# huang-yh/GaussianFormer

Measured on AMD Instinct MI355X. Metric: Gaussians/sec splatted into 200×200×16×18 voxel grid (fwd), higher is better.
Workload: dtype f32

## Files before the change

### gaussianformer_amd/csrc/splat_bwd_mfma.hip

```cpp
#include <algorithm>


#include "gf_common.hpp"
#include "splat_mfma.hpp"

#ifndef GF_TIMELINE
#define GF_TIMELINE 0
#endif

namespace gf {

constexpr int kBwdBigTableAt = kLongWords, kBwdBigTable = (kBwdBigCap - kBwdBigTableAt - 1) / 3;
static_assert(kBwdBigTableAt >= kWRow && kBwdBigTable >= 64, "the table sits past the layout words in use");

struct BwdMArgs {
    const float *pts;
    const float *records;
    const uint2 *boxes;
    const unsigned long long *bitmask;
    const float *out_grad;
    float *rows;
    float *means_grad, *opa_grad, *sem_grad, *cov_grad;
    const uint32_t *state;
    uint32_t *tile_counters;
// ... 218 lines not shown
            if (off >= per_col) { off -= per_col; col += 1; }
        }
    };

    uint32_t *ctr = a.tile_counters + 64 * xcd;
    const int nchunk = (a.nwords + 63) >> 6;
    int local = (int)(blockIdx.x >> 3);
    while (true) {
        const int logical = local;
        const int qs = (int)__umulhi((uint32_t)logical, m_ps);
        if (!(local < per_xcd && 8 * qs + xcd < a.nsx * a.nsy)) break;
        uint32_t claimed = 0u;
        const int s = 8 * qs + xcd, r = logical - qs * per_super;
        const int srow = a.nsy == 1 ? s : (int)__umulhi((uint32_t)s, m_nsy), scol = s - srow * a.nsy;
        const int Xw = srow * kSuper + 4 * (r & 1), Y0 = scol * kSuper + 4 * ((r >> 1) & 1), Zw = 8 * (r >> 2);
        if (Xw < a.H && Y0 < a.W) {
#if GF_TIMELINE
            unsigned long long tl[8] = {(unsigned long long)wall_clock64(), 0, 0, 0, 0, 0, 0, 0};
#endif
            const uint32_t published_len = use_lists ? a.list_len[s] : 0u;
            request_unit(s, Xw, Y0, Zw);
            if (dl_by16) asm volatile("s_waitcnt vmcnt(9)" ::: "memory");
            else asm volatile("s_waitcnt vmcnt(36)" ::: "memory");
#if GF_TIMELINE
            tl[1] = wall_clock64();
#endif
            int list_len = 0, qlen = 0, qhead = 0, npend = 0;
            int c = 0, sg = 0;
            bool have_boxes = false;
            const bool pub_unit = LONG ? (use_lists && published_len != 0xFFFFFFFFu) : use_lists;
            int pub_done = 0;
            bool pub_fetch = false;
            if (pub_unit) {
                list_len = min((int)published_len, kMList);
                c = nchunk;
                have_boxes = true;
            } else if (!LONG) {
                constexpr int kWDense = kMList;
                uint32_t *s_dw = s_u;
                unsigned long long *s_db = reinterpret_cast<unsigned long long *>(s_u + kWDense);
                constexpr int kWPer = (kWRow + 63) / 64;
                const int kw = nchunk;
                unsigned long long wd[kWPer];
                int mine = 0;
                int wlane = lane;
                asm volatile("" : "+v"(wlane));
                const int wbase = kw * wlane;
#pragma unroll
                for (int k = 0; k < kWPer; ++k) wd[k] = s_row[min(wbase + k, kWRow - 1)];
                static_assert(kWPer == 10, "operand list below");
                asm volatile("" : "+v"(wd[0]), "+v"(wd[1]), "+v"(wd[2]), "+v"(wd[3]), "+v"(wd[4]), "+v"(wd[5]), "+v"(wd[6]), "+v"(wd[7]),
                             "+v"(wd[8]), "+v"(wd[9]));
#pragma unroll
                for (int k = 0; k < kWPer; ++k) {
                    const int w = wbase + k;
                    wd[k] = (k < kw && w < a.nwords) ? wd[k] : 0ull;
                    mine += wd[k] != 0ull ? 1 : 0;
                }
                const int incl_nz = wave_incl_scan_dpp(mine);
                const int nd = __builtin_amdgcn_readlane(incl_nz, 63);
                if (nd <= kWDense) {
                    int p = incl_nz - mine;
#pragma unroll
                    for (int k = 0; k < kWPer; ++k) {
                        if (wd[k] != 0ull) {
                            s_dw[p] = (uint32_t)(wbase + k);
                            s_db[p] = wd[k];
// ... 754 lines not shown
```

### gaussianformer_amd/csrc/splat_fwd.hip

```cpp
#include <string.h>

#include <algorithm>

#include "gf_common.hpp"
#include "splat_mfma.hpp"

#ifndef GF_TIMELINE
#define GF_TIMELINE 0
#endif

namespace gf {

struct PrepArgs {
    const float *means3D;
    const int *means_int;
    const float *opacity;
    const float *semantics;
    const int *radii;
    const float *cov3D;
    const int *points_int;
    const float *pts;
    float *records;
    uint2 *boxes;
    unsigned long long *bitmask;
    uint32_t *verify_flags;
    int P, N, H, W, D, nwords, nrow, nsx, nsy, per_axis, variant, nprep_blocks, verify, prescale, exact_det, lattice;
    uint32_t *tile_counters;
    uint32_t tile_counter_init;
    uint32_t *unit_totals;
    uint32_t *unit_local;
    uint32_t *bwd_counters;
    uint32_t bwd_counter_init;
    uint32_t *gen_word;
    const uint32_t *gate_state;
    int range_theta_here;
    uint32_t *verdict_words;
    unsigned char *summary;
    int sum_pitch;
    uint32_t *range_flags;
};

constexpr int kPrepSuperChunk = 4096;

__device__ __forceinline__ void gaussian_box(const int *__restrict__ means_int, const int *__restrict__ radii,
                                             int per_axis, int g, int H, int W, int D, int lo[3], int hi[3])
{
    const int m0 = means_int[3 * g], m1 = means_int[3 * g + 1], m2 = means_int[3 * g + 2];
    int r0, r1, r2;
    if (per_axis) {
        r0 = radii[3 * g]; r1 = radii[3 * g + 1]; r2 = radii[3 * g + 2];
    } else {
        r0 = r1 = r2 = radii[g];
    }
    lo[0] = min(H, max(0, m0 - r0)); hi[0] = min(H, max(0, m0 + r0 + 1));
    lo[1] = min(W, max(0, m1 - r1)); hi[1] = min(W, max(0, m1 + r1 + 1));
    lo[2] = min(D, max(0, m2 - r2)); hi[2] = min(D, max(0, m2 + r2 + 1));
}

__device__ __forceinline__ float prob_kdet(float c0, float c1, float c2, float c3, float c4, float c5, int exact)
{
    float deter, kdet;
    prob_det_kdet(c0, c1, c2, c3, c4, c5, exact, deter, kdet);
    return kdet;
}

constexpr float kSemRangeMax = 64.f;

__device__ __forceinline__ uint32_t range_bits_of(const float *c, const float *sm, float opa, int r0, int r1, int r2, int H, int W,
                                                  int D, float lsx, float lsy, float lsz)
{
    const float ex = (float)(min(r0, H) + 3) * lsx, ey = (float)(min(r1, W) + 3) * lsy, ez = (float)(min(r2, D) + 5) * lsz;
    const float bound = 0.7213475f * (fabsf(c[0]) + fabsf(c[1]) + fabsf(c[2])) * (ex * ex + ey * ey + ez * ez);
// ... 75 lines not shown
                                         (double)pz[k] == p0z + (double)z[k] * sz);
                }
            }
        }
        if (first_round) {
            p0x = q0x; p0y = q0y; p0z = q0z;
            sx = a.H > 1 ? (double)q1x - p0x : 1.0;
            sy = a.W > 1 ? (double)q1y - p0y : 1.0;
            sz = a.D > 1 ? (double)q1z - p0z : 1.0;
        }
        if (a.lattice) {
            const float lx_ = fabsf((float)sx), ly_ = fabsf((float)sy), lz_ = fabsf((float)sz);
            const float zero[kC] = {0.f};
            if (has_g) rbits |= range_bits_of(c0, zero, 0.f, rr0, rr1, rr2, a.H, a.W, a.D, lx_, ly_, lz_) & kVerdictTheta;
#pragma nounroll
            for (int g = g0 + kVerifyBlocks * 64; g < a.P; g += kVerifyBlocks * 64) {
                const float *cv = a.cov3D + 6 * (size_t)g;
                const int r0 = a.radii[a.per_axis ? 3 * g : g], r1 = a.radii[a.per_axis ? 3 * g + 1 : g], r2 = a.radii[a.per_axis ? 3 * g + 2 : g];
                float c[6];
#pragma unroll
                for (int j = 0; j < 6; ++j) c[j] = cv[j];
                rbits |= range_bits_of(c, zero, 0.f, r0, r1, r2, a.H, a.W, a.D, lx_, ly_, lz_) & kVerdictTheta;
            }
        }
        const unsigned long long any = __builtin_amdgcn_ballot_w64(bad), any2 = __builtin_amdgcn_ballot_w64(bad_lattice),
                                 any3 = __builtin_amdgcn_ballot_w64((rbits & kVerdictTheta) != 0u);
        const uint32_t vbits = (any ? kVerdictPoint : 0u) | (any2 ? kVerdictLattice : 0u) | (any3 ? kVerdictTheta : 0u);
        if (lane == 0) a.verify_flags[vb] = vbits;
        if (a.verdict_words && vbits && lane == 0) atomicOr(a.verdict_words + verdict_slot_after(a.verdict_words[kVerdictA]), vbits);
        return;
    }
    if (a.tile_counters && blockIdx.x == 0 && threadIdx.x < 8) a.tile_counters[64 * threadIdx.x] = a.tile_counter_init;
    if (a.verdict_words && blockIdx.x == 0 && threadIdx.x == 0) a.verdict_words[kVerdictB] = a.verdict_words[kVerdictA] + 1u;
    const int word = blockIdx.x * WAVES + wave;
    const int g = word * 64 + lane;
    const bool valid = g < a.P;
    int lo[3] = {0, 0, 0}, hi[3] = {0, 0, 0};
    uint32_t range_bits = 0u;
    float lsx = 0.f, lsy = 0.f, lsz = 0.f;
    if (a.range_flags && a.range_theta_here) {
        const float p0x = a.pts[0], p0y = a.pts[1], p0z = a.pts[2];
        lsx = a.H > 1 ? fabsf(a.pts[3 * (size_t)a.W * a.D] - p0x) : 1.f;
        lsy = a.W > 1 ? fabsf(a.pts[3 * (size_t)a.D + 1] - p0y) : 1.f;
        lsz = a.D > 1 ? fabsf(a.pts[3 + 2] - p0z) : 1.f;
    }
    auto range_of = [&](const float *c, const float *sm, float opa, int r0, int r1, int r2) -> uint32_t {
        return range_bits_of(c, sm, opa, r0, r1, r2, a.H, a.W, a.D, lsx, lsy, lsz);
    };
    float c_in[6] = {0.f, 0.f, 0.f, 0.f, 0.f, 0.f}, sm_in[kC], mean_in[3] = {0.f, 0.f, 0.f}, opa_in = 0.f;
    if (!STAGED) {
        const int gc = min(g, a.P - 1);
        const int m0 = a.means_int[3 * gc], m1 = a.means_int[3 * gc + 1], m2 = a.means_int[3 * gc + 2];
        const int r0 = a.radii[a.per_axis ? 3 * gc : gc], r1 = a.radii[a.per_axis ? 3 * gc + 1 : gc],
                  r2 = a.radii[a.per_axis ? 3 * gc + 2 : gc];
        const float *cv = a.cov3D + 6 * (size_t)gc;
        const float *sm = a.semantics + (size_t)kC * gc;
#pragma unroll
        for (int j = 0; j < 6; ++j) c_in[j] = cv[j];
#pragma unroll
        for (int j = 0; j < kC; ++j) sm_in[j] = sm[j];
        mean_in[0] = a.means3D[3 * gc]; mean_in[1] = a.means3D[3 * gc + 1]; mean_in[2] = a.means3D[3 * gc + 2];
        opa_in = a.opacity[gc];
        {
            int mm0 = m0, mm1 = m1, mm2 = m2, q0 = r0, q1 = r1, q2 = r2;
            asm volatile("" : "+v"(mm0), "+v"(mm1), "+v"(mm2), "+v"(q0), "+v"(q1), "+v"(q2), "+v"(mean_in[0]), "+v"(mean_in[1]), "+v"(mean_in[2]), "+v"(opa_in),
                              "+v"(c_in[0]), "+v"(c_in[4]), "+v"(sm_in[0]), "+v"(sm_in[4]), "+v"(sm_in[8]), "+v"(sm_in[12]), "+v"(sm_in[16]));
// ... 218 lines not shown
}

struct RenderArgs {
    const float *pts;
    const int *points_int;
    const float *records;
    const uint2 *boxes;
    const unsigned long long *bitmask;
    float *out_logits;
    float *out_bin;
    float *out_density;
    float *out_prob;
    const uint32_t *verify_flags;
    uint32_t *state;
    unsigned long long *timeline;
    const int *tile_perm;
    int P, N, nwords, nrow, H, W, D, nsx, nsy, ntiles_total, verify_dense;
    long long *out_labels;
    int label_mode, empty_label;
    float threshold;
    int raw_numerator;
    uint32_t *tile_counters;
    const uint32_t *range_flags;
    int nrange4;
    uint32_t rows_valid;
    const uint32_t *unit_totals, *unit_local;
    uint32_t *unit_first;
    uint32_t unit_cap;
    uint32_t *pub_lists, *pub_len;
    uint32_t *verdict_words;
    const unsigned char *summary;
    int sum_pitch;
    uint32_t m_ps, m_nsy;
};

__device__ __forceinline__ void stamp_state(const RenderArgs &a, uint32_t rows_ready = 0u)
{
    a.state[kStateGen] = *flag_word_via_verify(a.verify_flags, kGenWord);
    a.state[kStateRows] = rows_ready;
}

constexpr int kRowLayoutBlocks = 64;
static_assert(kRowLayoutBlocks * ((kWRow + 63) / 64) >= kWRow, "every wave of Gaussians has a workgroup");
__device__ __forceinline__ bool finish_row_layout(const RenderArgs &a, uint32_t *s_base, int lane)
{
    const int nw = a.nwords;
    constexpr int kPer = (kWRow + 63) / 64;
    static_assert(kPer == 10, "operand lists below");
    uint32_t t[kPer], loc[kPer];
#pragma unroll
    for (int k = 0; k < kPer; ++k) t[k] = a.unit_totals[min(kPer * lane + k, nw - 1)];
#pragma unroll
    for (int j = 0; j < kPer; ++j) loc[j] = a.unit_local[min(64 * ((int)blockIdx.x + kRowLayoutBlocks * j) + lane, a.P - 1)];
    asm volatile("" : "+v"(t[0]), "+v"(t[1]), "+v"(t[2]), "+v"(t[3]), "+v"(t[4]), "+v"(t[5]), "+v"(t[6]), "+v"(t[7]), "+v"(t[8]), "+v"(t[9]));
    asm volatile("" : "+v"(loc[0]), "+v"(loc[1]), "+v"(loc[2]), "+v"(loc[3]), "+v"(loc[4]), "+v"(loc[5]), "+v"(loc[6]), "+v"(loc[7]), "+v"(loc[8]), "+v"(loc[9]));
    uint32_t mine = 0u;
#pragma unroll
    for (int k = 0; k < kPer; ++k) {
        t[k] = kPer * lane + k < nw ? (t[k] & 0x7FFFFFFFu) : 0u;
        mine += t[k];
    }
    const uint32_t incl = (uint32_t)wave_incl_scan_dpp((int)mine);
    const uint32_t total = (uint32_t)__builtin_amdgcn_readlane((int)incl, 63);
    uint32_t run = incl - mine;
#pragma unroll
    for (int k = 0; k < kPer; ++k) {
// ... 1030 lines not shown
    }
    return t;
}
__device__ const PhiHotTable kPhiHot = make_phi_hot_table();

constexpr int kWList = 512;
constexpr int kWLdsDwords = 5120;
static_assert(3072 + 2 * kWRow + kQCap + (kC + 1) * kSRow == kWLdsDwords, "LDS map of the wave-autonomous kernel");
static_assert((kWRow + 4 + 3) / 4 <= 3 * 64, "the wave kernel reads its range verdicts with three 16-byte loads per lane");
static_assert(2 * 64 * kC <= 1536 + 3 * kWList, "output staging fits over the slot and the list");

constexpr int kLDense = 576, kLIds = 896;
static_assert(2 * kLDense + kLDense / 2 <= 1536 && 1536 + 3 * kLIds <= 3072 + 2 * kWRow && kLDense % 64 == 0 && kLIds % 64 == 0 && kLIds == kBwdPubLong, "LDS map of the long-row instantiation");
constexpr int kLSumAt = 3968;
static_assert(kLSumAt == 1536 + 3 * kLIds - 64 * 4, "the summary row is the tail of box hi (LDS map above)");
static_assert(kLSumAt < kLongWords, "finish_row_layout_long's prefix reaches the summary row: the first unit re-fetches it past kLSumAt words");
static_assert(kLongWords <= 64 * 64, "one summary bit per word, 64 per lane");
template <bool LABELS, bool PREP = false, bool LONG = false>
__global__ __launch_bounds__(64, 2) void gf_splat_render_mfma_wave_kernel(RenderArgs a)
{
    __shared__ __attribute__((aligned(16))) uint32_t s_u[kWLdsDwords];
    float4 *slot = reinterpret_cast<float4 *>(s_u);
    constexpr int kListN = LONG ? kLIds : kWList;
    uint32_t *s_lg = s_u + 1536, *s_blo = s_u + 1536 + kListN, *s_bhi = s_u + 1536 + 2 * kListN;
    float *stage = reinterpret_cast<float *>(s_u);
    unsigned long long *s_row = reinterpret_cast<unsigned long long *>(s_u + 3072);
    uint32_t *s_sum = s_u + kLSumAt;
    uint32_t *q_id = s_u + 3072 + 2 * kWRow;
    float *S = reinterpret_cast<float *>(s_u + 3072 + 2 * kWRow + kQCap);

    const int lane = threadIdx.x;
    const int xcd = (int)(blockIdx.x & 7u);
    const int per_super = 4 * ((a.D + 7) >> 3);
    const int per_xcd = ((a.nsx * a.nsy + 7) >> 3) * per_super;

    const uint32_t m_ps = a.m_ps, m_nsy = a.m_nsy;
    int local = (int)(blockIdx.x >> 3);
    bool row_there = false;
    {
        const int q0 = (int)__umulhi((uint32_t)local, m_ps);
        if (local < per_xcd && 8 * q0 + xcd < a.nsx * a.nsy) {
            const int s0 = 8 * q0 + xcd, r0 = local - q0 * per_super;
            const int srow0 = a.nsy == 1 ? s0 : (int)__umulhi((uint32_t)s0, m_nsy), scol0 = s0 - srow0 * a.nsy;
            if (srow0 * kSuper + 4 * (r0 & 1) < a.H && scol0 * kSuper + 4 * ((r0 >> 1) & 1) < a.W) {
                if (LONG) {
                    lds_dma16((gptr)(a.summary + (size_t)s0 * a.sum_pitch + 16 * min(lane, (a.sum_pitch >> 4) - 1)), (lptr)s_sum);
                } else {
                    const unsigned long long *bm0 = a.bitmask + (size_t)s0 * a.nrow;
                    for (int i = 0; 128 * i < a.nrow; ++i)
                        if (128 * i + 2 * lane < a.nrow)
                            lds_dma16((gptr)(bm0 + 128 * i + 2 * lane), (lptr)(s_row + 128 * i));
                }
                row_there = true;
            }
        }
    }
    float q0x, q0y, q0z, q1x, q1y, q1z;
    {
        const float *pp = a.pts;
        asm volatile("" : "+v"(pp));
        const size_t ix = a.H > 1 ? 3 * (size_t)a.W * a.D : 0, iy = a.W > 1 ? 3 * (size_t)a.D + 1 : 1, iz = a.D > 1 ? 3 + 2 : 2;
        asm volatile("global_load_dword %0, %6, off\n\tglobal_load_dword %1, %6, off offset:4\n\tglobal_load_dword %2, %6, off offset:8\n\t"
                     "global_load_dword %3, %7, off\n\tglobal_load_dword %4, %8, off\n\tglobal_load_dword %5, %9, off"
                     : "=&v"(q0x), "=&v"(q0y), "=&v"(q0z), "=&v"(q1x), "=&v"(q1y), "=&v"(q1z)
                     : "v"(pp), "v"(pp + ix), "v"(pp + iy), "v"(pp + iz)
                     : "memory");
    }
    uint4 phihot_raw[8];
    {
        const uint4 *tp = reinterpret_cast<const uint4 *>(&kPhiHot.w[0][0][0]) + lane;
#pragma unroll
        for (int k = 0; k < 8; ++k) phihot_raw[k] = tp[64 * k];
    }
    int verdict = 0;
    if (a.verdict_words) {
        const uint4 vw = *reinterpret_cast<const uint4 *>(a.verdict_words);
        const uint32_t vv = (vw.y & 1u) ? vw.w : vw.z;
        verdict = __builtin_amdgcn_readfirstlane((int)(vv & (a.verify_dense ? kVerdictAll : kVerdictRange)));
        if (blockIdx.x == 0 && lane == 0) {
            a.verdict_words[kVerdictA] = vw.y;
            a.verdict_words[verdict_slot_after(vw.y)] = 0u;
        }
    } else {
        uint32_t v = 0u, rv = 0u;
        uint4 r0 = make_uint4(0, 0, 0, 0), r1 = r0, r2 = r0;
        if (a.range_flags) {
            const uint4 *rp = reinterpret_cast<const uint4 *>(a.range_flags);
            const int last = a.nrange4 - 1;
            r0 = rp[min(lane, last)]; r1 = rp[min(lane + 64, last)]; r2 = rp[min(lane + 128, last)];
        }
        if (a.verify_dense) {
            const uint4 *vp = reinterpret_cast<const uint4 *>(a.verify_flags) + 16 * lane;
#pragma unroll
            for (int k = 0; k < 16; ++k) {
                const uint4 t = vp[k];
                v |= t.x | t.y | t.z | t.w;
            }
        }
        rv = r0.x | r0.y | r0.z | r0.w | r1.x | r1.y | r1.z | r1.w | r2.x | r2.y | r2.z | r2.w;
        rv |= v;
        verdict = (__builtin_amdgcn_ballot_w64((v & kVerdictPoint) != 0u) ? kVerdictPoint : 0) | (__builtin_amdgcn_ballot_w64((v & kVerdictLattice) != 0u) ? kVerdictLattice : 0) |
                  (__builtin_amdgcn_ballot_w64((rv & kVerdictTheta) != 0u) ? kVerdictTheta : 0) | (__builtin_amdgcn_ballot_w64((rv & kVerdictOpaSem) != 0u) ? kVerdictOpaSem : 0);
    }
    asm volatile("s_waitcnt vmcnt(0)" : "+v"(q0x), "+v"(q0y), "+v"(q0z), "+v"(q1x), "+v"(q1y), "+v"(q1z)::"memory");
    uint32_t rows_ready = 0u;
    if (PREP && blockIdx.x < (unsigned)kRowLayoutBlocks && a.rows_valid && !verdict) {
        rows_ready = (LONG ? finish_row_layout_long(a, s_u, lane) : finish_row_layout(a, s_u, lane)) ? kRowsReady : kRowsOverflow;
        if (LONG && a.nwords > kLSumAt) row_there = false;
    }
    if (blockIdx.x == 0 && lane == 0 && a.state) {
        a.state[kStateNotDense] = (verdict & kVerdictPoint) ? 1u : 0u;
// ... 17 lines not shown
    q1z = __builtin_bit_cast(float, __builtin_amdgcn_readfirstlane(__builtin_bit_cast(int, q1z)));
    const double p0x = q0x, p0y = q0y, p0z = q0z;
    const double sx = a.H > 1 ? (double)q1x - p0x : 1.0;
    const double sy = a.W > 1 ? (double)q1y - p0y : 1.0;
    const double sz = a.D > 1 ? (double)q1z - p0z : 1.0;

    h8 phi[4], hot[4];
#pragma unroll
    for (int b = 0; b < 4; ++b) {
        phi[b] = __builtin_bit_cast(h8, phihot_raw[b]);
        hot[b] = __builtin_bit_cast(h8, phihot_raw[4 + b]);
    }

    auto request_records_at = [&](int qh, int start, int count) {
        const uint32_t id = q_id[(qh + start + (n < count ? n : 0)) & (kQCap - 1)];
        const char *rec = reinterpret_cast<const char *>(a.records + (size_t)id * kRecDwords);
        const int o3 = (3 + 2 * h) * 16, o4 = (4 + 2 * h) * 16, o5 = (5 + 2 * h) * 16;
        request_record_pieces(rec, reinterpret_cast<char *>(slot), o3, o4, o5);
    };

    uint32_t st_off[5];
#pragma unroll
    for (int j = 0; j < 5; ++j) {
        const int i = lane + 64 * j;
        const int run = i / kC, k = i - run * kC;
        st_off[j] = i < 16 * kC ? (uint32_t)(((((size_t)(run >> 2) * a.W + (run & 3)) * a.D) * kC + 4 * k) * sizeof(float)) : 0u;
    }
    const bool st_tail = lane + 64 * 4 < 16 * kC;
    const bool st_fits = (3 * (size_t)a.W + 4) * a.D * kC * sizeof(float) < ((size_t)1 << 32);

    uint32_t *ctr = a.tile_counters + 64 * xcd;
    const int nchunk = (a.nwords + 63) >> 6;
    int nst_prev = 0;
    while (true) {
        const int logical = local;
        const int qs = (int)__umulhi((uint32_t)logical, m_ps);
        if (!(local < per_xcd && 8 * qs + xcd < a.nsx * a.nsy)) break;
        bool next_row = false;
        int nst = -1;
        uint32_t claimed = 0u;
        bool have_next = false;
        const int s = 8 * qs + xcd, r = logical - qs * per_super;
        const int srow = a.nsy == 1 ? s : (int)__umulhi((uint32_t)s, m_nsy), scol = s - srow * a.nsy;
        const int Xw = srow * kSuper + 4 * (r & 1), Y0 = scol * kSuper + 4 * ((r >> 1) & 1), Zw = 8 * (r >> 2);
        if (Xw < a.H && Y0 < a.W) {
            const unsigned long long *__restrict__ bm = a.bitmask + (size_t)s * a.nrow;
#if GF_TIMELINE
            unsigned long long tl[8] = {(unsigned long long)wall_clock64(), 0, 0, 0, 0, 0, 0, 0};
#endif
            if (!row_there) {
                if (LONG) {
                    lds_dma16((gptr)(a.summary + (size_t)s * a.sum_pitch + 16 * min(lane, (a.sum_pitch >> 4) - 1)), (lptr)s_sum);
                } else {
                    for (int i = 0; 128 * i < a.nrow; ++i)
                        if (128 * i + 2 * lane < a.nrow)
                            lds_dma16((gptr)(bm + 128 * i + 2 * lane), (lptr)(s_row + 128 * i));
                }
            }
            f32x16 acc[4];
#pragma unroll
            for (int b = 0; b < 4; ++b)
#pragma unroll
                for (int q = 0; q < 16; ++q) acc[b][q] = 0.f;
            const double Cx = p0x + ((double)Xw + 1.5) * sx, Cy = p0y + ((double)Y0 + 1.5) * sy, Cz = p0z + ((double)Zw + 3.5) * sz;
            bool published = false;
            int list_len = 0, qlen = 0, qhead = 0, npend = 0;
            if (row_there && nst_prev == 10) asm volatile("s_waitcnt vmcnt(10)" ::: "memory");
            else asm volatile("s_waitcnt vmcnt(0)" ::: "memory");
#if GF_TIMELINE
            tl[1] = wall_clock64();
#endif
            int c = 0, sg = 0;
            int long_lo = 0;
            bool long_first = true;
            if (!LONG) {
                constexpr int kWDense = kWList;
                uint32_t *s_dw = s_u;
                unsigned long long *s_db = reinterpret_cast<unsigned long long *>(s_u + kWDense);
                constexpr int kWPer = (kWRow + 63) / 64;
                const int kw = nchunk;
                unsigned long long wd[kWPer];
                int mine = 0;
#pragma unroll
                for (int k = 0; k < kWPer; ++k) wd[k] = s_row[min(kw * lane + k, kWRow - 1)];
                static_assert(kWPer == 10, "operand list below");
                asm volatile("" : "+v"(wd[0]), "+v"(wd[1]), "+v"(wd[2]), "+v"(wd[3]), "+v"(wd[4]), "+v"(wd[5]), "+v"(wd[6]), "+v"(wd[7]),
                             "+v"(wd[8]), "+v"(wd[9]));
#pragma unroll
                for (int k = 0; k < kWPer; ++k) {
                    const int w = kw * lane + k;
                    wd[k] = (k < kw && w < a.nwords) ? wd[k] : 0ull;
                    mine += wd[k] != 0ull ? 1 : 0;
                }
                const int incl_nz = wave_incl_scan_dpp(mine);
                const int nd = __builtin_amdgcn_readlane(incl_nz, 63);
                if (nd <= kWDense) {
                    int p = incl_nz - mine;
#pragma unroll
                    for (int k = 0; k < kWPer; ++k) {
                        if (wd[k] != 0ull) {
                            s_dw[p] = (uint32_t)(kw * lane + k);
                            s_db[p] = wd[k];
                            ++p;
                        }
                    }
                }
                if (nd <= kWDense) {
                    __builtin_amdgcn_fence(__ATOMIC_ACQ_REL, "wavefront");
// ... 29 lines not shown
                        }
#pragma unroll
                        for (int q = 0; q < 3; ++q) in_[q] = wave_incl_scan_dpp(cn[q]);
#pragma unroll
                        for (int q = 0; q < 3; ++q) tt[q] = __builtin_amdgcn_readlane(in_[q], 63);
                        tot = tt[0] + tt[1] + tt[2];
                        if (tot <= kWList) {
                            extract(bb[0], ii[0], in_[0] - cn[0]);
                            extract(bb[1], ii[1], tt[0] + in_[1] - cn[1]);
                            extract(bb[2], ii[2], tt[0] + tt[1] + in_[2] - cn[2]);
                        } else {
                            fits = false;
                        }
                    } else {
                        for (int d0 = 0; d0 < nd; d0 += 64) {
                            const int i = d0 + lane;
                            const unsigned long long bits = i < nd ? s_db[i] : 0ull;
                            const uint32_t id0 = (i < nd ? s_dw[i] : 0u) * 64u;
                            const int cnt = __builtin_popcountll(bits);
                            const int incl = wave_incl_scan_dpp(cnt);
                            const int t = __builtin_amdgcn_readlane(incl, 63);
                            if (tot + t > kWList) {
                                fits = false;
                                break;
                            }
                            extract(bits, id0, tot + incl - cnt);
                            tot += t;
                        }
                    }
                    if (fits) {
                        list_len = tot;
                        c = nchunk;
                    }
                }
            }
            while (true) {
                bool last = false;
                if (LONG) {
                    uint32_t *d_lo = s_u, *d_hi = s_u + kLDense;
                    unsigned short *d_w = reinterpret_cast<unsigned short *>(s_u + 2 * kLDense);
                    if (!long_first) {
                        lds_dma16((gptr)(a.summary + (size_t)s * a.sum_pitch + 16 * min(lane, (a.sum_pitch >> 4) - 1)), (lptr)s_sum);
                        asm volatile("s_waitcnt vmcnt(0)" ::: "memory");
                    }
                    long_first = false;
                    const uint4 sv = reinterpret_cast<const uint4 *>(s_sum)[lane];
                    auto nib16 = [](uint32_t d) -> uint32_t {
                        uint32_t x = d & 0x0F0F0F0Fu;
                        x = (x | (x >> 4)) & 0x00FF00FFu;
                        return (x | (x >> 8)) & 0x0000FFFFu;
                    };
                    unsigned long long sm = (unsigned long long)(nib16(sv.x) | (nib16(sv.y) << 16)) |
                                            ((unsigned long long)(nib16(sv.z) | (nib16(sv.w) << 16)) << 32);
                    {
                        const int left = a.nwords - 64 * lane;
                        sm = left >= 64 ? sm : (left > 0 ? sm & bits_below(left) : 0ull);
                    }
                    const int cw = __builtin_popcountll(sm);
                    const int incl_w = wave_incl_scan_dpp(cw);
                    const int nd = __builtin_amdgcn_readlane(incl_w, 63);
                    const int cnt = min(nd - long_lo, kLDense);
                    {
                        unsigned long long m = sm;
                        int t = incl_w - cw - long_lo;
                        while (m) {
                            const int b = __builtin_ctzll(m);
// ... 82 lines not shown
                                full = true;
                                break;
                            }
                            if ((lane >> 3) == sg) pos = list_len + (incl - cnt) - e0;
                            list_len += e1 - e0;
                        }
                        if (!full) {
                            sg = 0;
                            ++c;
                        }
                        if (pos >= 0) {
                            const uint32_t id0 = (uint32_t)w * 64u;
                            while (bits) {
                                const int j = __builtin_ctzll(bits);
                                bits &= bits - 1;
                                s_lg[pos++] = id0 + (uint32_t)j;
                            }
                        }
                        if (full) break;
                        continue;
                    }
                    const uint32_t id0 = (uint32_t)w * 64u;
                    while (bits) {
                        const int j = __builtin_ctzll(bits);
                        bits &= bits - 1;
                        s_lg[pos++] = id0 + (uint32_t)j;
                    }
                }
                __builtin_amdgcn_fence(__ATOMIC_ACQ_REL, "wavefront");
                __builtin_amdgcn_wave_barrier();
#if GF_TIMELINE
                if (!tl[2]) tl[2] = wall_clock64();
#endif
                for (int b0 = 0; b0 < list_len; b0 += 64) {
                    const uint32_t id = s_lg[min(b0 + lane, list_len - 1)];
                    lds_dma4((gptr)(&a.boxes[id].x), (lptr)(s_blo + b0));
                    lds_dma4((gptr)(&a.boxes[id].y), (lptr)(s_bhi + b0));
                }
                asm volatile("s_waitcnt vmcnt(0)" ::: "memory");
                if (PREP && a.rows_valid && r == 0 && !published) {
                    published = true;
                    constexpr int kPub = LONG ? kBwdPubLong : kBwdList;
                    if (last && list_len <= kPub) {
                        uint32_t *dst = a.pub_lists + (size_t)s * (3 * kPub);
                        for (int i = lane; i < list_len; i += 64) {
                            dst[i] = s_lg[i]; dst[kPub + i] = s_blo[i]; dst[2 * kPub + i] = s_bhi[i];
                        }
                        if (lane == 0) a.pub_len[s] = (uint32_t)list_len;
                    } else if (lane == 0) {
                        if (LONG) a.pub_len[s] = 0xFFFFFFFFu;
                        else atomicOr(const_cast<uint32_t *>(flag_word_via_verify(a.verify_flags, kListsBad)), 1u);
                    }
                }
#if GF_TIMELINE
                if (!tl[3]) tl[3] = wall_clock64();
#endif
                const int nbase = list_len + ((LONG && !last) ? 64 : 0);
                for (int base = 0; base < nbase || (last && base == 0); base += 64) {
                    const int i = base + lane;
                    const int ic = min(i, max(list_len - 1, 0));
                    const uint32_t eg = s_lg[ic];
                    const uint32_t blo = s_blo[ic], bhi = s_bhi[ic];
                    const bool hit = i < list_len && ux(blo) < Xw + 4 && ux(bhi) > Xw && uy(blo) < Y0 + 4 && uy(bhi) > Y0 &&
                                     uz(blo) < Zw + 8 && uz(bhi) > Zw;
                    const unsigned long long todo = __builtin_amdgcn_ballot_w64(hit);
                    if (hit) q_id[(qhead + qlen + (int)mbcnt(todo)) & (kQCap - 1)] = eg;
                    qlen += __builtin_popcountll(todo);
                    const bool final_batch = last && base + 64 >= list_len;
                    const bool flush = LONG && !last && base >= list_len;
                    while (true) {
                        if (npend == 0) {
                            if (!(qlen >= 32 || (final_batch && qlen > 0))) break;
                            npend = min(qlen, 32);
                            __builtin_amdgcn_fence(__ATOMIC_ACQ_REL, "wavefront");
                            __builtin_amdgcn_wave_barrier();
                            request_records_at(qhead, 0, npend);
                        }
                        const int avail = qlen - npend;
                        if (!(avail >= 32 || final_batch || flush)) break;
                        const int qn = npend;
                        asm volatile("s_waitcnt vmcnt(0)" ::: "memory");
#if GF_TIMELINE
                        if (!tl[4]) tl[4] = wall_clock64();
                        tl[7] += 1;
// ... 57 lines not shown
                        __builtin_amdgcn_wave_barrier();
                        H8 sh[2], sl[2];
#pragma unroll
                        for (int q = 0; q < 4; ++q) {
                            const float4 v4 = *reinterpret_cast<const float4 *>(S + min(n, kC) * kSRow + 8 * q + 4 * h);
                            const fp16x2 ha = __builtin_amdgcn_cvt_pkrtz(v4.x, v4.y), hb = __builtin_amdgcn_cvt_pkrtz(v4.z, v4.w);
                            float ra0, ra1, rb0, rb1;
                            asm("v_fma_mix_f32 %0, %1, -1.0, %2 op_sel_hi:[1,0,0]" : "=v"(ra0) : "v"(ha), "v"(v4.x));
                            asm("v_fma_mix_f32 %0, %1, -1.0, %2 op_sel:[1,0,0] op_sel_hi:[1,0,0]" : "=v"(ra1) : "v"(ha), "v"(v4.y));
                            asm("v_fma_mix_f32 %0, %1, -1.0, %2 op_sel_hi:[1,0,0]" : "=v"(rb0) : "v"(hb), "v"(v4.z));
                            asm("v_fma_mix_f32 %0, %1, -1.0, %2 op_sel:[1,0,0] op_sel_hi:[1,0,0]" : "=v"(rb1) : "v"(hb), "v"(v4.w));
                            sh[q >> 1].p[2 * (q & 1)] = ha; sh[q >> 1].p[2 * (q & 1) + 1] = hb;
                            sl[q >> 1].p[2 * (q & 1)] = __builtin_amdgcn_cvt_pkrtz(ra0, ra1); sl[q >> 1].p[2 * (q & 1) + 1] = __builtin_amdgcn_cvt_pkrtz(rb0, rb1);
                        }
                        exp_accumulate_pair(t1, t2, t3, tb, phi[0], phi[1], hot[0], hot[1], sh, sl, acc[0], acc[1]);
                        exp_accumulate_pair(t1, t2, t3, tb, phi[2], phi[3], hot[2], hot[3], sh, sl, acc[2], acc[3]);
                        have_next = have_next || last_group;
                        qhead = (qhead + qn) & (kQCap - 1);
                        qlen -= qn;
                        npend = nnext;
                    }
                }
                if (last) break;
                list_len = 0;
            }
#if GF_TIMELINE
            asm volatile("" :: "v"(acc[0]), "v"(acc[1]), "v"(acc[2]), "v"(acc[3]));
            tl[5] = wall_clock64();
#endif
            if (!have_next && lane == 0)
                asm volatile("global_atomic_add %0, %1, %2, off sc0" : "=v"(claimed) : "v"(ctr), "v"(1u) : "memory");
            asm volatile("s_waitcnt vmcnt(0)" : "+v"(claimed)::"memory");
            have_next = true;
            {
                const int nl = __builtin_amdgcn_readfirstlane((int)claimed);
                const int q2 = (int)__umulhi((uint32_t)nl, m_ps);
                if (nl < per_xcd && 8 * q2 + xcd < a.nsx * a.nsy) {
                    const int s2 = 8 * q2 + xcd, r2 = nl - q2 * per_super;
                    const int srow2 = a.nsy == 1 ? s2 : (int)__umulhi((uint32_t)s2, m_nsy), scol2 = s2 - srow2 * a.nsy;
                    if (srow2 * kSuper + 4 * (r2 & 1) < a.H && scol2 * kSuper + 4 * ((r2 >> 1) & 1) < a.W) {
                        if (LONG) {
                            lds_dma16((gptr)(a.summary + (size_t)s2 * a.sum_pitch + 16 * min(lane, (a.sum_pitch >> 4) - 1)), (lptr)s_sum);
                        } else {
                            const unsigned long long *bm2 = a.bitmask + (size_t)s2 * a.nrow;
                            for (int i = 0; 128 * i < a.nrow; ++i)
                                if (128 * i + 2 * lane < a.nrow)
                                    lds_dma16((gptr)(bm2 + 128 * i + 2 * lane), (lptr)(s_row + 128 * i));
                        }
                        next_row = true;
                    }
                }
            }
            if ((a.D & 3) == 0) {
#pragma unroll
                for (int b = 0; b < 4; ++b) {
                    float *row = stage + ((b >> 1) * 64 + 32 * (b & 1) + n) * kC;
                    *reinterpret_cast<float2 *>(row + 4 * h) = make_float2(acc[b][0], acc[b][1]);
                    *reinterpret_cast<float2 *>(row + 4 * h + 2) = make_float2(acc[b][2], acc[b][3]);
                    *reinterpret_cast<float2 *>(row + 8 + 4 * h) = make_float2(acc[b][4], acc[b][5]);
                    *reinterpret_cast<float2 *>(row + 10 + 4 * h) = make_float2(acc[b][6], acc[b][7]);
                    if (h == 0) *reinterpret_cast<float2 *>(row + 16) = make_float2(acc[b][8], acc[b][9]);
                }
                auto labels_from_stage = [&]() {
#pragma unroll
                    for (int half = 0; half < 2; ++half) {
                        const int l = lane;
                        const float *row = stage + (64 * half + l) * kC;
                        float best = row[0];
                        int arg = 0;
#pragma unroll
                        for (int ch = 1; ch < kC; ++ch) {
                            const float v = row[ch];
                            if (v > best) { best = v; arg = ch; }
                        }
                        const int cx = Xw + (l >> 4), cy = Y0 + ((l >> 2) & 3), cz = Zw + 4 * half + (l & 3);
                        if (cx < a.H && cy < a.W && cz < a.D) a.out_labels[((size_t)cx * a.W + cy) * a.D + cz] = arg;
                    }
                };
                if (LABELS) {
                    __builtin_amdgcn_fence(__ATOMIC_ACQ_REL, "wavefront");
// ... 279 lines not shown

static int splat_forward_impl(const char *fn, int variant, int flags, int C, const gf::SplatInputs &in, const gf::ForwardOutputs &out,
                              void *workspace, size_t workspace_bytes, void *stream_)
{
    using namespace gf;
    hipStream_t stream = (hipStream_t)stream_;
    const int *label_mode = out.labels ? &out.label_mode : nullptr;
    if (int rc = check_splat_shape(fn, variant, C, in)) return rc;
    GF_CHECK_ARG_AS(fn, in.N == 0 || (in.pts && in.points_int && (out.logits || out.labels)), "null point/output pointer");
    GF_CHECK_ARG_AS(fn, in.P == 0 || (in.means3D && in.means3D_int && in.opacity && in.semantics && in.radii && in.cov3D),
                    "null Gaussian pointer");
    GF_CHECK_ARG_AS(fn, variant == GF_SPLAT_BASE || in.N == 0 || (out.bin_logits && out.density && out.probability) ||
                            (out.labels && !out.logits && !out.bin_logits && !out.density && !out.probability),
                    "prob variant needs bin_logits/density/probability outputs (all three, or none in labels-only mode)");
    if (int rc = check_forward_modes(fn, variant, flags, label_mode)) return rc;
    GF_CHECK_ARG_AS(fn, workspace != nullptr, "null workspace");
    const SplatWorkspace ws = carve_workspace(workspace, in.P, in.N, in.H, in.W, in.D);
    if (workspace_bytes < ws.total_bytes) {
        set_error("%s: workspace too small (%zu < %zu)", fn, workspace_bytes, ws.total_bytes);
        return GF_EWORKSPACE;
    }
    const ForwardRoute rt = forward_route(variant, flags, label_mode, in, ws);
    uint32_t *const tile_counters = ws.flags + kFwdCounters;
    uint32_t *const verdict_words = rt.one_verdict ? ws.flags + kVerdictWords : nullptr;
    unsigned char *const summary = rt.summaries ? ws.summary : nullptr;

    PrepArgs pa = fill_prep_args(in, ws);
    pa.variant = variant; pa.nprep_blocks = rt.prep_blocks; pa.verify = rt.verify; pa.prescale = rt.prescale;
    pa.exact_det = (flags & GF_PROB_EXACT_DET) ? 1 : 0; pa.lattice = rt.lattice;
    pa.unit_totals = rt.row_layout ? ws.bwd_wave_total : nullptr; pa.bwd_counter_init = rt.bwd_counter_init;
    pa.tile_counters = rt.range_flags ? tile_counters : nullptr; pa.tile_counter_init = rt.tile_counter_init;
    pa.range_flags = rt.range_flags ? ws.range_flags : nullptr; pa.range_theta_here = rt.range_theta_here;
    pa.verdict_words = verdict_words; pa.summary = summary; pa.sum_pitch = ws.sum_pitch;
    if (rt.prep_grid > 0) {
        launch_prep(pa, rt.prep_waves == 4, rt.prep_grid, stream);
        GF_CHECK_LAUNCH_AS(fn);
    }
    if (in.N == 0) return GF_OK;

    RenderArgs ra;
    ra.pts = in.pts; ra.points_int = in.points_int; ra.records = ws.records; ra.boxes = ws.boxes; ra.bitmask = ws.bitmask;
    ra.out_logits = out.logits; ra.out_bin = out.bin_logits; ra.out_density = out.density; ra.out_prob = out.probability;
    ra.verify_flags = ws.flags + kVerifyBase; ra.state = (uint32_t *)out.state; ra.P = in.P; ra.N = in.N; ra.nwords = ws.nwords; ra.nrow = ws.nrow;
    ra.H = in.H; ra.W = in.W; ra.D = in.D; ra.nsx = ws.nsx; ra.nsy = ws.nsy; ra.ntiles_total = ws.nsuper * kTilesPerSuper;
    ra.verify_dense = rt.verify;
    ra.timeline = g_timeline;
    ra.tile_perm = g_tile_perm;
    ra.out_labels = out.labels; ra.label_mode = out.label_mode; ra.empty_label = out.empty_label; ra.threshold = out.threshold;
    ra.raw_numerator = (flags & GF_PROB_NUMERATOR) ? 1 : 0;
    ra.tile_counters = tile_counters;
    ra.range_flags = pa.range_flags;
    ra.nrange4 = (ws.nwords + 3) / 4;
    ra.rows_valid = rt.row_layout ? 1u : 0u;
    ra.unit_totals = ws.bwd_wave_total; ra.unit_local = ws.bwd_row_local; ra.unit_first = ws.bwd_row_first; ra.unit_cap = ws.bwd_cap;
    ra.pub_lists = ws.bwd_lists; ra.pub_len = ws.bwd_list_len;
    ra.verdict_words = verdict_words;
    ra.summary = summary; ra.sum_pitch = ws.sum_pitch;
    ra.m_ps = ceil_recip32(splat_units(1, in.D)); ra.m_nsy = ceil_recip32(ws.nsy);
    hipEvent_t ev0, ev1;
    const bool prof = rt.kernel != kRenderArbitrary && profile_slot(&ev0, &ev1);
    if (prof) (void)hipEventRecord(ev0, stream);
    if (rt.kernel >= kRenderMfmaTile) launch_render_mfma(rt, ra, stream);
    else if (variant == GF_SPLAT_BASE) rt.labels ? launch_render_exact<GF_SPLAT_BASE, true>(rt, ra, stream) : launch_render_exact<GF_SPLAT_BASE, false>(rt, ra, stream);
    else rt.labels ? launch_render_exact<GF_SPLAT_PROB, true>(rt, ra, stream) : launch_render_exact<GF_SPLAT_PROB, false>(rt, ra, stream);
    if (prof) (void)hipEventRecord(ev1, stream);
    GF_CHECK_LAUNCH_AS(fn);
    return GF_OK;
}

extern "C" int gf_splat_forward(int variant, int radii_per_axis, int flags, int P, int N, int C, int H,
                                int W, int D, const float *pts, const int *points_int,
                                const float *means3D, const int *means3D_int, const float *opacity,
                                const float *semantics, const int *radii, const float *cov3D,
                                float *out_logits, float *out_bin_logits, float *out_density,
                                float *out_probability, void *state, void *workspace,
                                size_t workspace_bytes, void *stream)
{
    const gf::SplatInputs in{radii_per_axis ? 1 : 0, P, N, H, W, D, pts, means3D, opacity, semantics, cov3D, points_int, means3D_int, radii};
    const gf::ForwardOutputs out{out_logits, out_bin_logits, out_density, out_probability, nullptr, 0, 0, 0.f, state};
    return splat_forward_impl(__func__, variant, flags, C, in, out, workspace, workspace_bytes, stream);
}

extern "C" int gf_splat_forward_labels(int variant, int radii_per_axis, int flags, int P, int N, int C, int H,
                                       int W, int D, const float *pts, const int *points_int,
                                       const float *means3D, const int *means3D_int, const float *opacity,
                                       const float *semantics, const int *radii, const float *cov3D,
                                       float *out_logits, float *out_bin_logits, float *out_density,
                                       float *out_probability, int label_mode, float threshold, int empty_label,
                                       long long *out_labels, void *state, void *workspace, size_t workspace_bytes,
                                       void *stream)
{
// ... 23 lines not shown
```

Baseline: 703.4 million.

## Share per-supertile Gaussian lists across units within a forward pass

```diff
diff --git a/gaussianformer_amd/csrc/splat_bwd_mfma.hip b/gaussianformer_amd/csrc/splat_bwd_mfma.hip
--- a/gaussianformer_amd/csrc/splat_bwd_mfma.hip
+++ b/gaussianformer_amd/csrc/splat_bwd_mfma.hip
@@ -274,7 +274,7 @@
             int pub_done = 0;
             bool pub_fetch = false;
             if (pub_unit) {
-                list_len = min((int)published_len, kMList);
+                list_len = min((int)(LONG ? published_len : (published_len & 0xFFFFu)), kMList);
                 c = nchunk;
                 have_boxes = true;
             } else if (!LONG) {
diff --git a/gaussianformer_amd/csrc/splat_fwd.hip b/gaussianformer_amd/csrc/splat_fwd.hip
--- a/gaussianformer_amd/csrc/splat_fwd.hip
+++ b/gaussianformer_amd/csrc/splat_fwd.hip
@@ -38,6 +38,7 @@
     unsigned char *summary;
     int sum_pitch;
     uint32_t *range_flags;
+    uint32_t *pub_len;
 };
 
 constexpr int kPrepSuperChunk = 4096;
@@ -179,6 +180,8 @@
     }
     if (a.tile_counters && blockIdx.x == 0 && threadIdx.x < 8) a.tile_counters[64 * threadIdx.x] = a.tile_counter_init;
     if (a.verdict_words && blockIdx.x == 0 && threadIdx.x == 0) a.verdict_words[kVerdictB] = a.verdict_words[kVerdictA] + 1u;
+    if (a.pub_len && blockIdx.x == 0)
+        for (int i = threadIdx.x; i < a.nsx * a.nsy; i += 64 * WAVES) a.pub_len[i] = 0u;
     const int word = blockIdx.x * WAVES + wave;
     const int g = word * 64 + lane;
     const bool valid = g < a.P;
@@ -463,6 +466,7 @@
     const unsigned char *summary;
     int sum_pitch;
     uint32_t m_ps, m_nsy;
+    uint32_t m_nx;
 };
 
 __device__ __forceinline__ void stamp_state(const RenderArgs &a, uint32_t rows_ready = 0u)
@@ -1559,15 +1563,30 @@
     const int lane = threadIdx.x;
     const int xcd = (int)(blockIdx.x & 7u);
     const int per_super = 4 * ((a.D + 7) >> 3);
-    const int per_xcd = ((a.nsx * a.nsy + 7) >> 3) * per_super;
-
-    const uint32_t m_ps = a.m_ps, m_nsy = a.m_nsy;
+    const int nsuper_xcd = (a.nsx * a.nsy + 7) >> 3;
+    const int per_xcd = nsuper_xcd * per_super;
+
+    const uint32_t m_ps = a.m_ps, m_nsy = a.m_nsy, m_nx = a.m_nx;
+    auto unit_qr = [&](int u, int &q, int &r) {
+        if (LONG) {
+            q = (int)__umulhi((uint32_t)u, m_ps);
+            r = u - q * per_super;
+        } else if (u < nsuper_xcd) {
+            q = u;
+            r = 0;
+        } else {
+            const int v = u - nsuper_xcd;
+            q = (int)__umulhi((uint32_t)v, m_nx);
+            r = 1 + v - q * (per_super - 1);
+        }
+    };
     int local = (int)(blockIdx.x >> 3);
     bool row_there = false;
     {
-        const int q0 = (int)__umulhi((uint32_t)local, m_ps);
+        int q0, r0;
+        unit_qr(local, q0, r0);
         if (local < per_xcd && 8 * q0 + xcd < a.nsx * a.nsy) {
-            const int s0 = 8 * q0 + xcd, r0 = local - q0 * per_super;
+            const int s0 = 8 * q0 + xcd;
             const int srow0 = a.nsy == 1 ? s0 : (int)__umulhi((uint32_t)s0, m_nsy), scol0 = s0 - srow0 * a.nsy;
             if (srow0 * kSuper + 4 * (r0 & 1) < a.H && scol0 * kSuper + 4 * ((r0 >> 1) & 1) < a.W) {
                 if (LONG) {
@@ -1600,10 +1619,12 @@
         for (int k = 0; k < 8; ++k) phihot_raw[k] = tp[64 * k];
     }
     int verdict = 0;
+    uint32_t pub_tag = 0u;
     if (a.verdict_words) {
         const uint4 vw = *reinterpret_cast<const uint4 *>(a.verdict_words);
         const uint32_t vv = (vw.y & 1u) ? vw.w : vw.z;
         verdict = __builtin_amdgcn_readfirstlane((int)(vv & (a.verify_dense ? kVerdictAll : kVerdictRange)));
+        if (!LONG) pub_tag = (uint32_t)__builtin_amdgcn_readfirstlane((int)(((vw.y & 0x7FFFu) | 0x8000u) << 16));
         if (blockIdx.x == 0 && lane == 0) {
             a.verdict_words[kVerdictA] = vw.y;
             a.verdict_words[verdict_slot_after(vw.y)] = 0u;
@@ -1687,15 +1708,17 @@
     uint32_t *ctr = a.tile_counters + 64 * xcd;
     const int nchunk = (a.nwords + 63) >> 6;
     int nst_prev = 0;
+    bool pl_there = false;
     while (true) {
         const int logical = local;
-        const int qs = (int)__umulhi((uint32_t)logical, m_ps);
+        int qs, r;
+        unit_qr(logical, qs, r);
         if (!(local < per_xcd && 8 * qs + xcd < a.nsx * a.nsy)) break;
         bool next_row = false;
         int nst = -1;
         uint32_t claimed = 0u;
         bool have_next = false;
-        const int s = 8 * qs + xcd, r = logical - qs * per_super;
+        const int s = 8 * qs + xcd;
         const int srow = a.nsy == 1 ? s : (int)__umulhi((uint32_t)s, m_nsy), scol = s - srow * a.nsy;
         const int Xw = srow * kSuper + 4 * (r & 1), Y0 = scol * kSuper + 4 * ((r >> 1) & 1), Zw = 8 * (r >> 2);
         if (Xw < a.H && Y0 < a.W) {
@@ -1726,9 +1749,29 @@
             tl[1] = wall_clock64();
 #endif
             int c = 0, sg = 0;
+            bool have_boxes = false;
+            if (!LONG && pl_there) {
+                const uint32_t plv = (uint32_t)__builtin_amdgcn_readfirstlane((int)q_id[0]);
+                if ((plv & 0xFFFF0000u) == pub_tag && (plv & 0xFFFFu) <= (uint32_t)kBwdList) {
+                    int wl = lane;
+                    asm volatile("" : "+v"(wl));
+                    const uint32_t *src = a.pub_lists + (size_t)s * (3 * kBwdList) + 4 * wl;
+                    lds_dma16((gptr)src, (lptr)s_lg);
+                    lds_dma16((gptr)(src + kBwdList), (lptr)s_blo);
+                    lds_dma16((gptr)(src + 2 * kBwdList), (lptr)s_bhi);
+                    if (lane == 0) asm volatile("global_atomic_add %0, %1, off" ::"v"(ctr + 32), "v"(1u) : "memory");
+                    asm volatile("s_waitcnt vmcnt(0)" ::: "memory");
+                    list_len = (int)(plv & 0xFFFFu);
+                    c = nchunk;
+                    have_boxes = true;
+#if GF_TIMELINE
+                    tl[7] += 1000;
+#endif
+                }
+            }
             int long_lo = 0;
             bool long_first = true;
-            if (!LONG) {
+            if (!LONG && !have_boxes) {
                 constexpr int kWDense = kWList;
                 uint32_t *s_dw = s_u;
                 unsigned long long *s_db = reinterpret_cast<unsigned long long *>(s_u + kWDense);
@@ -1824,6 +1867,34 @@
                         list_len = tot;
                         c = nchunk;
                     }
+                }
+            }
+            const bool for_backward = PREP && a.rows_valid;
+            if (!LONG && r == 0 && (for_backward || pub_tag != 0u)) {
+                if (c >= nchunk && list_len <= kBwdList) {
+                    __builtin_amdgcn_fence(__ATOMIC_ACQ_REL, "wavefront");
+                    __builtin_amdgcn_wave_barrier();
+                    int wl = lane;
+                    asm volatile("" : "+v"(wl));
+                    for (int b0 = 0; b0 < list_len; b0 += 64) {
+                        const uint32_t id = s_lg[min(b0 + wl, list_len - 1)];
+                        lds_dma4((gptr)(&a.boxes[id].x), (lptr)(s_blo + b0));
+                        lds_dma4((gptr)(&a.boxes[id].y), (lptr)(s_bhi + b0));
+                    }
+                    asm volatile("s_waitcnt vmcnt(0)" ::: "memory");
+                    have_boxes = true;
+                    uint32_t *dst = a.pub_lists + (size_t)s * (3 * kBwdList);
+                    for (int i = wl; i < list_len; i += 64) {
+                        dst[i] = s_lg[i]; dst[kBwdList + i] = s_blo[i]; dst[2 * kBwdList + i] = s_bhi[i];
+                    }
+                    uint32_t word = (uint32_t)list_len;
+                    if (pub_tag != 0u) {
+                        asm volatile("s_waitcnt vmcnt(0)" ::: "memory");
+                        word |= pub_tag;
+                    }
+                    if (wl == 0) a.pub_len[s] = word;
+                } else if (for_backward && lane == 0) {
+                    atomicOr(const_cast<uint32_t *>(flag_word_via_verify(a.verify_flags, kListsBad)), 1u);
                 }
             }
             while (true) {
@@ -1972,24 +2043,23 @@
 #if GF_TIMELINE
                 if (!tl[2]) tl[2] = wall_clock64();
 #endif
-                for (int b0 = 0; b0 < list_len; b0 += 64) {
+                for (int b0 = 0; b0 < list_len && !have_boxes; b0 += 64) {
                     const uint32_t id = s_lg[min(b0 + lane, list_len - 1)];
                     lds_dma4((gptr)(&a.boxes[id].x), (lptr)(s_blo + b0));
                     lds_dma4((gptr)(&a.boxes[id].y), (lptr)(s_bhi + b0));
                 }
+                have_boxes = false;
                 asm volatile("s_waitcnt vmcnt(0)" ::: "memory");
-                if (PREP && a.rows_valid && r == 0 && !published) {
+                if (LONG && PREP && a.rows_valid && r == 0 && !published) {
                     published = true;
-                    constexpr int kPub = LONG ? kBwdPubLong : kBwdList;
-                    if (last && list_len <= kPub) {
-                        uint32_t *dst = a.pub_lists + (size_t)s * (3 * kPub);
+                    if (last && list_len <= kBwdPubLong) {
+                        uint32_t *dst = a.pub_lists + (size_t)s * (3 * kBwdPubLong);
                         for (int i = lane; i < list_len; i += 64) {
-                            dst[i] = s_lg[i]; dst[kPub + i] = s_blo[i]; dst[2 * kPub + i] = s_bhi[i];
+                            dst[i] = s_lg[i]; dst[kBwdPubLong + i] = s_blo[i]; dst[2 * kBwdPubLong + i] = s_bhi[i];
                         }
                         if (lane == 0) a.pub_len[s] = (uint32_t)list_len;
                     } else if (lane == 0) {
-                        if (LONG) a.pub_len[s] = 0xFFFFFFFFu;
-                        else atomicOr(const_cast<uint32_t *>(flag_word_via_verify(a.verify_flags, kListsBad)), 1u);
+                        a.pub_len[s] = 0xFFFFFFFFu;
                     }
                 }
 #if GF_TIMELINE
@@ -2113,11 +2183,13 @@
                 asm volatile("global_atomic_add %0, %1, %2, off sc0" : "=v"(claimed) : "v"(ctr), "v"(1u) : "memory");
             asm volatile("s_waitcnt vmcnt(0)" : "+v"(claimed)::"memory");
             have_next = true;
+            pl_there = false;
             {
                 const int nl = __builtin_amdgcn_readfirstlane((int)claimed);
-                const int q2 = (int)__umulhi((uint32_t)nl, m_ps);
+                int q2, r2;
+                unit_qr(nl, q2, r2);
                 if (nl < per_xcd && 8 * q2 + xcd < a.nsx * a.nsy) {
-                    const int s2 = 8 * q2 + xcd, r2 = nl - q2 * per_super;
+                    const int s2 = 8 * q2 + xcd;
                     const int srow2 = a.nsy == 1 ? s2 : (int)__umulhi((uint32_t)s2, m_nsy), scol2 = s2 - srow2 * a.nsy;
                     if (srow2 * kSuper + 4 * (r2 & 1) < a.H && scol2 * kSuper + 4 * ((r2 >> 1) & 1) < a.W) {
                         if (LONG) {
@@ -2127,6 +2199,11 @@
                             for (int i = 0; 128 * i < a.nrow; ++i)
                                 if (128 * i + 2 * lane < a.nrow)
                                     lds_dma16((gptr)(bm2 + 128 * i + 2 * lane), (lptr)(s_row + 128 * i));
+                            if (pub_tag != 0u && r2 != 0) {
+                                const uint32_t *lp = a.pub_len + s2;
+                                asm volatile("s_mov_b32 m0, %1\n\ts_nop 0\n\tglobal_load_lds_dword %0, off sc1" ::"v"(lp), "s"((uint32_t)(uintptr_t)(lptr)q_id) : "memory", "m0");
+                                pl_there = true;
+                            }
                         }
                         next_row = true;
                     }
@@ -2472,6 +2549,7 @@
     pa.tile_counters = rt.range_flags ? tile_counters : nullptr; pa.tile_counter_init = rt.tile_counter_init;
     pa.range_flags = rt.range_flags ? ws.range_flags : nullptr; pa.range_theta_here = rt.range_theta_here;
     pa.verdict_words = verdict_words; pa.summary = summary; pa.sum_pitch = ws.sum_pitch;
+    pa.pub_len = (rt.kernel == kRenderMfmaWave && verdict_words) ? ws.bwd_list_len : nullptr;
     if (rt.prep_grid > 0) {
         launch_prep(pa, rt.prep_waves == 4, rt.prep_grid, stream);
         GF_CHECK_LAUNCH_AS(fn);
@@ -2497,6 +2575,7 @@
     ra.verdict_words = verdict_words;
     ra.summary = summary; ra.sum_pitch = ws.sum_pitch;
     ra.m_ps = ceil_recip32(splat_units(1, in.D)); ra.m_nsy = ceil_recip32(ws.nsy);
+    ra.m_nx = ceil_recip32(splat_units(1, in.D) - 1);
     hipEvent_t ev0, ev1;
     const bool prof = rt.kernel != kRenderArbitrary && profile_slot(&ev0, &ev1);
     if (prof) (void)hipEventRecord(ev0, stream);
```

After: 723.6 million (median of 6 runs). 1.03x the previous value.
